# Ashish424/G.P.U-PathTracer

Hardware: AMD Instinct MI355X
Metric: Mrays/sec, cornell_dragon 1920x1080 (+ achieved GB/s against the memory roofline) (higher is better)
Workload: dtype f32; 1 GPU; cornell_dragon_800k (800032 tris) 1920x1080 depth 4 diff + reference 8-sphere room, 16 spp per step; kernel=auto, parallelism=1 GPU, closed_scene=True

## Files before the change

g.p.u-pathtracer_amd/__init__.py:

```python
from . import _abi
from ._abi import (Camera, Params, Sphere, Material, Counters, BuildParams, DenoiseParams, MAT_DIFF, MAT_METAL, MAT_SPEC, MAT_REFR,
                   FLAG_METAL_LITERAL_W, FLAG_WRITE_RGBA, FLAG_FACE_FORWARD, FLAG_COSINE_DIFF, FLAG_GLASS_FIX, FLAG_RUSSIAN_ROULETTE, FLAG_MISS_KEEPS_PATH, FLAG_RR_CPU_TRACER, FLAG_NEE, FLAGS_SMALLPT, FLAGS_CPU_TRACER, KERNEL_AUTO, KERNEL_MEGA_BVH2,
                   KERNEL_PERSISTENT, KERNEL_WAVEFRONT, OPT_KERNEL, OPT_COUNTERS, OPT_TIMING, OPT_BATCH, OPT_TOP_NODES, OPT_OCCUPANCY, OPT_LDS_STACK, OPT_WALK, OPT_LEAF_MAX, OPT_TRI_TEST, OPT_REFILL, OPT_VOTE_NODE, OPT_VOTE_REC, OPT_WAVE_BATCH, OPT_SPHERE_LDS, OPT_BUILD_ALGO, OPT_REBUILD, OPT_PRESPLIT, OPT_WAVE_BLOCKS, OPT_OVERLAP, OPT_OPTIMIZE, OPT_WAVE_SAMPLES,
                   OPT_FIRST_WALK, OPT_PACKET_STACK, OPT_FUSE_STAGES)
from .host import (Mesh, Bvh, write_image, save_checkpoint, load_checkpoint, frame_hash, reference_spheres, default_camera, default_params, scene_mesh)
from .tracer import PathTracer, PtError, DeviceBuffer, algorithmic_bytes, DENOISE_DEFAULTS

__all__ = [n for n in dir() if not n.startswith("_")]
```

g.p.u-pathtracer_amd/_abi.py:

```python
import ctypes as C
import os

_HERE = os.path.dirname(os.path.abspath(__file__))
PTMI_PATH = os.environ.get("PT_LIBPTMI") or os.path.join(_HERE, "csrc", "libptmi.so")
PTHOST_PATH = os.path.join(_HERE, "host", "libpthost.so")


class Camera(C.Structure):
    _fields_ = [("pos", C.c_float * 3), ("front", C.c_float * 3), ("right", C.c_float * 3),
                ("up", C.c_float * 3), ("dist", C.c_float), ("aspect", C.c_float),
                ("fov", C.c_float), ("_pad", C.c_float)]


class Sphere(C.Structure):
    _fields_ = [("pos_rad", C.c_float * 4), ("emi", C.c_float * 3), ("col", C.c_float * 3),
                ("mat", C.c_int32)]


class Material(C.Structure):
    _fields_ = [("col", C.c_float * 3), ("emi", C.c_float * 3), ("mat", C.c_int32), ("phong_expo", C.c_float)]


class DenoiseParams(C.Structure):
    _fields_ = [("width", C.c_int32), ("height", C.c_int32), ("iterations", C.c_int32),
# ... 22 lines not shown

class BuildParams(C.Structure):
    _fields_ = [("max_leaf_size", C.c_int32), ("min_leaf_size", C.c_int32), ("max_depth", C.c_int32),
                ("n_bins", C.c_int32), ("sah_node_cost", C.c_float), ("sah_tri_cost", C.c_float),
                ("split_alpha", C.c_float), ("n_spatial_bins", C.c_int32), ("optimize_passes", C.c_int32)]


class BvhStats(C.Structure):
    _fields_ = [("n_inner", C.c_uint64), ("n_leaves", C.c_uint64), ("n_tri_refs", C.c_uint64),
                ("max_depth", C.c_uint32), ("sah_cost", C.c_float), ("build_ms", C.c_double),
                ("opt_cost_before", C.c_float), ("opt_cost_after", C.c_float)]


MAT_DIFF, MAT_METAL, MAT_SPEC, MAT_REFR = 0, 1, 2, 3
FLAG_METAL_LITERAL_W = 1 << 0
FLAG_WRITE_RGBA = 1 << 1
FLAG_FACE_FORWARD, FLAG_COSINE_DIFF, FLAG_GLASS_FIX, FLAG_RUSSIAN_ROULETTE, FLAG_MISS_KEEPS_PATH = 1 << 2, 1 << 3, 1 << 4, 1 << 5, 1 << 6
FLAG_RR_CPU_TRACER = 1 << 7
FLAG_NEE = 1 << 8
FLAGS_SMALLPT = FLAG_FACE_FORWARD | FLAG_COSINE_DIFF | FLAG_RUSSIAN_ROULETTE | FLAG_MISS_KEEPS_PATH
FLAGS_CPU_TRACER = FLAG_FACE_FORWARD | FLAG_COSINE_DIFF | FLAG_RR_CPU_TRACER | FLAG_MISS_KEEPS_PATH
KERNEL_AUTO, KERNEL_MEGA_BVH2, KERNEL_PERSISTENT, KERNEL_WAVEFRONT = 0, 1, 3, 5
OPT_KERNEL, OPT_COUNTERS, OPT_TIMING, OPT_BATCH, OPT_TOP_NODES, OPT_OCCUPANCY, OPT_LDS_STACK, OPT_WALK, OPT_LEAF_MAX, OPT_TRI_TEST, OPT_REFILL, OPT_VOTE_NODE, OPT_VOTE_REC, OPT_WAVE_BATCH, OPT_SPHERE_LDS, OPT_BUILD_ALGO, OPT_REBUILD, OPT_PRESPLIT, OPT_WAVE_BLOCKS, OPT_OVERLAP, OPT_OPTIMIZE, OPT_WAVE_SAMPLES = 1, 2, 3, 4, 5, 6, 7, 8, 9, 10, 11, 12, 13, 14, 15, 16, 17, 18, 19, 21, 24, 25
OPT_FIRST_WALK, OPT_PACKET_STACK, OPT_FUSE_STAGES = 26, 27, 28

_vp, _sz, _i, _u32 = C.c_void_p, C.c_size_t, C.c_int, C.c_uint32
PTMI_SYMBOLS = [
    ("pt_abi_version", _i, []),
    ("pt_device_count", _i, []),
    ("pt_create", _i, [_i, C.POINTER(_vp)]),
    ("pt_destroy", _i, [_vp]),
    ("pt_last_error", C.c_char_p, [_vp]),
    ("pt_set_stream", _i, [_vp, _vp]),
    ("pt_set_option", _i, [_vp, _i, _i]),
    ("pt_sync", _i, [_vp]),
    ("pt_malloc", _i, [_vp, _sz, C.POINTER(_vp)]),
    ("pt_free", _i, [_vp, _vp]),
    ("pt_memset", _i, [_vp, _vp, _i, _sz]),
    ("pt_download", _i, [_vp, _vp, _vp, _sz]),
    ("pt_upload", _i, [_vp, _vp, _vp, _sz]),
    ("pt_upload_bvh", _i, [_vp, _vp, _sz, _vp, _sz, _vp, _sz]),
    ("pt_upload_spheres", _i, [_vp, C.POINTER(Sphere), _sz]),
    ("pt_render", _i, [_vp, _vp, _vp, C.POINTER(Camera), C.POINTER(Params), _u32]),
    ("pt_trace_rays", _i, [_vp, _vp, _sz, _i, _vp, _vp, _vp]),
    ("pt_render_aux", _i, [_vp, C.POINTER(Camera), C.POINTER(Params), _vp, _vp, _vp, _vp]),
    ("pt_denoise", _i, [_vp, C.POINTER(DenoiseParams), _vp, _vp, _vp, _vp, _vp, _vp]),
    ("pt_build_bvh", _i, [_vp, _vp, C.c_size_t, _vp, C.c_size_t]),
# ... 78 lines not shown
```

g.p.u-pathtracer_amd/csrc/pt_ctx.h:

```cpp
#pragma once
#include <hip/hip_runtime.h>

#include <algorithm>
#include <cstdint>
#include <string>
#include <vector>

#include "../../include/ptmi.h"
#include "pt_kernels.h"

#ifndef PT_FIRST_WALK_DEFAULT
#define PT_FIRST_WALK_DEFAULT 1
#endif

struct pt_ctx {
    int device = 0;
    hipStream_t own_stream = nullptr;
    hipStream_t stream = nullptr;
    std::string err;
    float4* d_nodes = nullptr;
    float4* d_tris = nullptr;
    pt_sphere_d* d_spheres = nullptr;
    int* d_tri_matid = nullptr;
    float4* d_mat_table = nullptr;
// ... 28 lines not shown
    int opt_presplit = 0;
    int opt_optimize = 0;
    double opt_cost[2] = {0.0, 0.0};
    int opt_rebuild = 0;
    int opt_build_algo = 1;
    int opt_sph_lds = 1;
    int opt_vote_node = 1, opt_vote_rec = 1;
    int opt_refill = 8;
    int opt_top = 64;
    int opt_occ = 6;
    int opt_lstk = 16;
    int opt_walk = 2;
    int opt_leaf_max = 2;
    int opt_tri_test = 0;
    bool records_woop = false;
    void* d_wave = nullptr;
    size_t wave_bytes = 0;
    int opt_wave_batch = 16;
    int opt_wave_samples = 16;
    int opt_wave_blocks = 8;
    int opt_first_walk = PT_FIRST_WALK_DEFAULT;
    int opt_packet_stack = PT_PACKET_STACK_MAX;
    int opt_fuse_stages = 1;
    struct AutoPick {
        static constexpr int TRIALS = 4, PENDING = 4, DECIDED = 5;
        uint64_t key = 0;
        int phase = 0;
        int choice = PT_KERNEL_PERSISTENT;
        hipEvent_t e[2 * TRIALS] = {nullptr, nullptr, nullptr, nullptr, nullptr, nullptr, nullptr, nullptr};
        float ms[2] = {0.f, 0.f};
        uint64_t used = 0;
    };
    static constexpr int N_PICKS = 8;
    AutoPick picks[N_PICKS];
    int pick_last = -1;
    uint64_t pick_tick = 0;
    uint64_t scene_gen = 0;
    uint64_t geom_gen = 0;
    hipEvent_t geom_ev = nullptr;
    struct Refit {
        uint64_t scene_gen = 0;
        const float4* items = nullptr;
        void* d_mem = nullptr;
        int4* bin_list = nullptr;
        int4* wide_list = nullptr;
        float* bin_box = nullptr;
// ... 94 lines not shown
```

g.p.u-pathtracer_amd/csrc/pt_k_wave.hip:

```cpp
#include "pt_ctx.h"

__device__ __forceinline__ int wf_block_rank(bool keep, int& total, int* s_cnt) {
    const unsigned long long m = __ballot(keep);
    const int w = threadIdx.x >> 6;
    const int in_wave = (int)__builtin_amdgcn_mbcnt_hi((uint32_t)(m >> 32), __builtin_amdgcn_mbcnt_lo((uint32_t)m, 0u));
    if ((threadIdx.x & 63) == 0) s_cnt[w] = __popcll(m);
    __syncthreads();
    int base = 0, tot = 0;
#pragma unroll
    for (int k = 0; k < PT_BLOCK / 64; k++) {
        const int c = s_cnt[k];
        if (k < w) base += c;
        tot += c;
    }
    total = tot;
    return base + in_wave;
}

__device__ __forceinline__ void wf_sphere_table() {
    if (threadIdx.x < 11 * PT_KSPHERES) {
        PT_KARGS(K);
        const float v = ((const __attribute__((address_space(4))) float*)&K.ksph[0])[threadIdx.x];
        ((float*)s_dyn)[threadIdx.x] = v;
        if (threadIdx.x % 11 < 4) ((float*)s_dyn)[88 + 4 * (threadIdx.x / 11) + threadIdx.x % 11] = v;
    }
    __syncthreads();
}

__global__ void __launch_bounds__(256) k_wf_prepare(const KParams P) {
    for (uint32_t i = threadIdx.x; i < P.spp; i += 256) P.wf.hashes[i] = pt_wang64(P.frame + i);
    for (uint32_t i = threadIdx.x; i < P.wf.queues_words; i += 256) P.wf.queues_all[i] = 0u;
}

__device__ __forceinline__ bool wf_slot_pixel(const KParams& P, uint32_t slot, uint32_t& s_idx, int& px, int& py) {
    if (slot >= P.wf.n_slots) return false;
    return pt_slot_pixel(P, slot, s_idx, px, py);
}

template <bool COUNT, int OCC, int LSTK, bool FIRST>
__global__ void __launch_bounds__(PT_BLOCK, OCC) k_wf_extend(const KParams P) {
    const int tid = threadIdx.x;
    const int lane = tid & 63;
    TravOverflow<LSTK> stk_ovf;
    TravStack<LSTK, PT_BLOCK> stk(__builtin_amdgcn_readfirstlane(tid & ~63), stk_ovf);
    const bool cull = P.cull != 0;
    const uint32_t n_regions = (uint32_t)P.wf.n_regions;
    const uint32_t shard_regions = (n_regions + PT_SHARDS - 1) / PT_SHARDS;
    const int batch = P.batch;

    uint32_t next = 0, end = 0;
    bool empty = false;
    int shard = (int)(blockIdx.x & (PT_SHARDS - 1));

    bool live = false;
    uint32_t idx = 0;
    v3 o = V3(0.f, 0.f, 0.f), d = V3(0.f, 0.f, 0.f);
    TravState ts;
    ts.idx = ts.idy = ts.idz = ts.oodx = ts.oody = ts.oodz = 0.f;
    ts.node = PT_SENTINEL; ts.leaf = 0; ts.sp = 0;
    ts.h.t = PT_F32_MAX; ts.h.tri = -1; ts.h.rec = 0;
    TravCount tc;
    tc.inner = tc.tris = tc.leaves = 0;
// ... 9 lines not shown
            uint32_t served = 0;
            for (int round = 0; round < 8 && served < (uint32_t)n_idle; round++) {
                if (next == end) {
                    bool got = false;
                    for (int tries = 0; tries < PT_SHARDS && !got; tries++) {
                        uint32_t k = 0;
                        if (lane == 0) k = atomicAdd(P.wf.queue + shard * PT_SHARD_STRIDE, 1u);
                        k = (uint32_t)__builtin_amdgcn_readfirstlane((int)k);
                        const uint32_t r = k * PT_SHARDS + (uint32_t)shard;
                        if (k < shard_regions && r < n_regions) {
                            next = r * PT_REGION;
                            if (FIRST) end = min(next + (uint32_t)PT_REGION, P.wf.n_slots);
                            else end = next + (uint32_t)__builtin_amdgcn_readfirstlane(P.wf.cnt_in[r]);
                            got = true;
                        } else {
                            shard = (shard + 1) & (PT_SHARDS - 1);
                        }
                    }
                    if (!got) { empty = true; break; }
                }
                const uint32_t take = min((uint32_t)n_idle - served, end - next);
                if (!live && rank >= served && rank < served + take) {
                    idx = next + (rank - served);
                    if (FIRST) {
                        uint32_t s_idx = 0;
                        int px = 0, py = 0;
                        if (wf_slot_pixel(P, idx, s_idx, px, py)) {
                            PathState ps;
                            path_begin_hashed(P, px, py, (uint64_t)((uint32_t)py * (uint32_t)P.W + (uint32_t)px), P.wf.hashes[s_idx], ps);
                            o = ps.o;
                            d = ps.d;
                            live = true;
                        }
                    } else {
                        const float4 a = pt_sld4(P.wf.ray0_in + idx), b = pt_sld4(P.wf.ray1_in + idx);
                        o = V3(a.x, a.y, a.z);
                        d = V3(a.w, b.x, b.y);
                        live = true;
                    }
                    if (live) trav_begin(ts, o, d, stk, P.sc.wide_root);
                }
                next += take;
                served += take;
            }
            if (COUNT && served) { it_begin++; act_begin += served; }
        }
        const unsigned long long busy = __ballot(live);
        if (!busy) {
            if (empty) break;
            continue;
        }
        const int n_dead = empty ? 64 - __popcll(busy) : 0;
        if (live) {
            const bool fin = trav_run_wide<COUNT, true, false, true>(ts, P.sc, o, d, cull, stk, tc, n_dead, batch);
            if (fin) {
                pt_sst2(P.wf.hit + idx, make_float2(ts.h.t, __int_as_float(ts.h.rec)));
                live = false;
                if (COUNT) n_rays++;
            }
        }
    }

    if (COUNT) {
        const uint32_t a = wave_sum_u32(n_rays), b = wave_sum_u32(tc.inner), c = wave_sum_u32(tc.tris), dd = wave_sum_u32(tc.leaves);
        const uint32_t w_it_node = wave_sum_u32(tc.it_node), w_act_node = wave_sum_u32(tc.act_node);
        const uint32_t w_it_rec = wave_sum_u32(tc.it_rec), w_act_rec = wave_sum_u32(tc.act_rec);
        const uint32_t w_ovf = wave_sum_u32(stk.n_ovf);
        if (lane == 0) {
            atomicAdd(&P.counters[0], (unsigned long long)a);
            atomicAdd(&P.counters[1], (unsigned long long)b);
            atomicAdd(&P.counters[2], (unsigned long long)c);
            atomicAdd(&P.counters[3], (unsigned long long)dd);
            atomicAdd(&P.counters[6], (unsigned long long)w_it_node);
            atomicAdd(&P.counters[7], (unsigned long long)w_act_node);
            atomicAdd(&P.counters[8], (unsigned long long)w_it_rec);
            atomicAdd(&P.counters[9], (unsigned long long)w_act_rec);
            atomicAdd(&P.counters[12], (unsigned long long)it_begin);
            atomicAdd(&P.counters[13], (unsigned long long)act_begin);
            atomicAdd(&P.counters[14], (unsigned long long)it_loop);
            atomicAdd(&P.counters[15], (unsigned long long)w_ovf);
        }
    }
}

template <bool COUNT>
__global__ void __launch_bounds__(PT_BLOCK, 8) k_wf_extend_packet(const KParams P) {
    const uint32_t n_groups = P.wf.n_slots / 64u;
    const uint32_t stride = gridDim.x * (uint32_t)(PT_BLOCK / 64);
    TravCount tc;
    tc.inner = tc.tris = tc.leaves = 0;
    tc.it_node = tc.act_node = tc.it_rec = tc.act_rec = 0;
    uint32_t n_rays = 0, n_walked = 0;
    for (uint32_t group = (uint32_t)__builtin_amdgcn_readfirstlane((int)(blockIdx.x * (PT_BLOCK / 64) + (threadIdx.x >> 6)));
         group < n_groups; group += stride) {
        const uint32_t slot = group * 64u + (threadIdx.x & 63u);
        uint32_t s_idx = 0;
        int px = 0, py = 0;
        v3 o = V3(0.f, 0.f, 0.f), d = V3(0.f, 0.f, 0.f);
        const bool in = wf_slot_pixel(P, slot, s_idx, px, py);
// ... 47 lines not shown
        return false;
    }
    v3 col;
    const bool done = LAST ? true : path_shade_hit(P, ps, h, sh, tri_n, col, 0, NEE ? req : nullptr);
    if (LAST) col = path_last_emission(P, ps, h, sh, 0);
    const v3 e = done ? col : ps.accu;
    if (FIRST) {
        pt_sst3(smp, V3(0.f + e.x, 0.f + e.y, 0.f + e.z));
    } else if (!(e.x == 0.f) || !(e.y == 0.f) || !(e.z == 0.f)) {
        smp[0] += e.x; smp[1] += e.y; smp[2] += e.z;
    }
    return !done;
}

template <int LP>
__device__ __forceinline__ void wf_fold_region(const KParams& P, uint32_t region) {
    if (threadIdx.x >= 64) return;
    uint32_t s_idx = 0;
    int px = 0, py = 0;
    const bool in = wf_slot_pixel(P, region * PT_REGION + (threadIdx.x / LP) * (4u * LP), s_idx, px, py);
    pt_fold_pixel_grouped<LP>(P, in, in ? (size_t)py * (size_t)P.W + (size_t)px : 0, (int)(threadIdx.x % LP));
}

template <bool COUNT, bool NEE, bool FIRST, bool LAST = false, int FOLD = 0>
__global__ void __launch_bounds__(PT_BLOCK) k_wf_shade(const KParams P) {
    __shared__ int s_cnt[PT_BLOCK / 64];
    __shared__ int s_cnt2[PT_BLOCK / 64];
    const uint32_t region = blockIdx.x;
    const int n_in = FIRST ? PT_REGION : P.wf.cnt_in[region];
    const bool last = LAST || P.wf.bounce + 1 >= P.depth;
    if (n_in == 0) {
        if (!last && threadIdx.x == 0) P.wf.cnt_out[region] = 0;
        if (NEE && threadIdx.x == 0) P.wf.s_cnt[region] = 0;
        if constexpr (FOLD > 0) wf_fold_region<FOLD>(P, region);
        return;
    }
    wf_sphere_table();
    const size_t i = (size_t)region * PT_REGION + threadIdx.x;
    bool have = (int)threadIdx.x < n_in;
    bool alive = false, tri_hit = false;
    PathState ps;
    NeeReq req;
    req.want = false;
    uint32_t pix = 0, s_idx = 0;
    int px = 0, py = 0;
    if (FIRST) have = wf_slot_pixel(P, (uint32_t)i, s_idx, px, py);
    if (have) {
// ... 11 lines not shown
                ps.nee_mask = (pix >> 24) | ((sn >> 31) << 8);
                pix &= 0xffffffu;
                sn &= 0x7fffffffu;
            }
            s_idx = sn >> 12;
            ps.mask = V3(pt_sld1(P.wf.mask_in + i), pt_sld1(P.wf.mask_in + (size_t)P.wf.cap + i), pt_sld1(P.wf.mask_in + 2 * (size_t)P.wf.cap + i));
            ps.accu = V3(0.f, 0.f, 0.f);
            ps.depth = P.wf.bounce;
            ps.rng = pt_rng_init(P.wf.hashes[s_idx], (uint64_t)pix);
            ps.rng.n = sn & 0xfffu;
        }
        const float2 hh = pt_sld2(P.wf.hit + i);
        Hit h;
        h.t = hh.x;
        h.rec = __float_as_int(hh.y);
        h.tri = -1;
        tri_hit = h.t < PT_F32_MAX;
        if (tri_hit) {
            h.tri = 0;
            if (P.tri_matid) h.tri = __float_as_int(P.sc.nodes[h.rec].w);
        }
        alive = wf_shade_segment<NEE, FIRST, LAST>(P, ps, h, tri_hit, pt_sample_ptr(P, s_idx, (size_t)pix), &req);
    }
    if (COUNT) {
        const uint32_t nh = wave_sum_u32(tri_hit ? 1u : 0u), np = wave_sum_u32(have && !alive ? 1u : 0u);
        if ((threadIdx.x & 63) == 0) {
            atomicAdd(&P.counters[4], (unsigned long long)nh);
            atomicAdd(&P.counters[5], (unsigned long long)np);
        }
    }
    if (NEE) {
        int n_sh;
        const int rs = wf_block_rank(req.want, n_sh, s_cnt2);
        if (req.want) {
            const size_t j = (size_t)region * PT_REGION + (size_t)rs;
            P.wf.s_ray0[j] = make_float4(req.o.x, req.o.y, req.o.z, req.d.x);
            P.wf.s_ray1[j] = make_float4(req.d.y, req.d.z, __uint_as_float(pix), __uint_as_float(s_idx));
            P.wf.s_con[j] = make_float4(req.contrib.x, req.contrib.y, req.contrib.z, req.t_max);
        }
        if (threadIdx.x == 0) P.wf.s_cnt[region] = n_sh;
    }
    if (last) {
        if constexpr (FOLD > 0) {
            __syncthreads();
            wf_fold_region<FOLD>(P, region);
        }
        return;
    }
    int total;
    const int r = PT_SURVIVOR_RANK(P, alive, ps, total, s_cnt);
    if (alive) {
        const size_t j = (size_t)region * PT_REGION + (size_t)r;
        pt_sst4(P.wf.ray0_out + j, make_float4(ps.o.x, ps.o.y, ps.o.z, ps.d.x));
        pt_sst4(P.wf.ray1_out + j, make_float4(ps.d.y, ps.d.z, __uint_as_float(NEE ? (pix | ((ps.nee_mask & 0xffu) << 24)) : pix),
                                              __uint_as_float((s_idx << 12) | ps.rng.n | (NEE ? (ps.nee_mask >> 8) << 31 : 0u))));
        pt_sst1(P.wf.mask_out + j, ps.mask.x);
        pt_sst1(P.wf.mask_out + (size_t)P.wf.cap + j, ps.mask.y);
        pt_sst1(P.wf.mask_out + 2 * (size_t)P.wf.cap + j, ps.mask.z);
    }
    if (threadIdx.x == 0) P.wf.cnt_out[region] = total;
}

__global__ void __launch_bounds__(PT_BLOCK, 8) k_wf_extend_packet_shade(const KParams P) {
    __shared__ int s_cnt[PT_BLOCK / 64];
    wf_sphere_table();
    const uint32_t region = blockIdx.x;
    const size_t i = (size_t)region * PT_REGION + threadIdx.x;
    uint32_t s_idx = 0;
    int px = 0, py = 0;
    const bool have = wf_slot_pixel(P, (uint32_t)i, s_idx, px, py);
    const uint32_t pix = (uint32_t)py * (uint32_t)P.W + (uint32_t)px;
    PathState ps;
    ps.o = ps.d = V3(0.f, 0.f, 0.f);
    if (have) path_begin_hashed(P, px, py, (uint64_t)pix, P.wf.hashes[s_idx], ps);
    TravCount tc;
    tc.inner = tc.tris = tc.leaves = 0;
    tc.it_node = tc.act_node = tc.it_rec = tc.act_rec = 0;
    Hit h = trav_packet_wide<false>(P.sc, ps.o, ps.d, P.cull != 0, have, tc);
    bool alive = false;
    if (have) {
        const bool tri_hit = h.t < PT_F32_MAX;
        if (tri_hit && !P.tri_matid) h.tri = 0;
        alive = wf_shade_segment<false, true, false>(P, ps, h, tri_hit, pt_sample_ptr(P, s_idx, (size_t)pix), nullptr);
    }
    if (P.wf.bounce + 1 >= P.depth) return;
    int total;
    const int r = PT_SURVIVOR_RANK(P, alive, ps, total, s_cnt);
    if (alive) {
        const size_t j = (size_t)region * PT_REGION + (size_t)r;
        pt_sst4(P.wf.ray0_out + j, make_float4(ps.o.x, ps.o.y, ps.o.z, ps.d.x));
        pt_sst4(P.wf.ray1_out + j, make_float4(ps.d.y, ps.d.z, __uint_as_float(pix), __uint_as_float((s_idx << 12) | ps.rng.n)));
        pt_sst1(P.wf.mask_out + j, ps.mask.x);
        pt_sst1(P.wf.mask_out + (size_t)P.wf.cap + j, ps.mask.y);
        pt_sst1(P.wf.mask_out + 2 * (size_t)P.wf.cap + j, ps.mask.z);
    }
    if (threadIdx.x == 0) P.wf.cnt_out[region] = total;
}

__global__ void __launch_bounds__(PT_BLOCK) k_wf_resolve(const KParams P) {
    const int n_in = P.wf.s_cnt[blockIdx.x];
    if ((int)threadIdx.x >= n_in) return;
    const size_t i = (size_t)blockIdx.x * PT_REGION + threadIdx.x;
    const float4 c = P.wf.s_con[i];
    const float2 hh = P.wf.s_hit[i];
    if (hh.x < c.w) return;
    const float4 b = P.wf.s_ray1[i];
    const uint32_t pix = __float_as_uint(b.z), s_idx = __float_as_uint(b.w);
    float* smp = pt_sample_ptr(P, s_idx, (size_t)pix);
    smp[0] += c.x; smp[1] += c.y; smp[2] += c.z;
}

namespace ptmi {

struct WaveLayout {
    size_t n_regions, cap, b_ray, b_mask, b_hit, b_cnt, b_hash, q_words, b_q, b_nee, need;
    bool nee;
};
// ... 71 lines not shown
        P.wf.s_con = (float4*)(base + 2 * b_ray);
        P.wf.s_hit = (float2*)(base + 3 * b_ray);
        P.wf.s_cnt = (int*)(base + 3 * b_ray + b_hit);
    }

    hipStream_t st = c->stream;
    P.sc.n_top = 0;
    P.sph_tab = 0;
    P.batch = c->opt_wave_batch;
    P.wf.hit = hit;
    P.wf.hashes = hashes;
    P.wf.queues_all = queues;
    P.wf.queues_words = (uint32_t)q_words;
    P.wf.cap = (uint32_t)cap;
    P.wf.n_regions = (int)n_regions;
    P.wf.n_slots = (uint32_t)((size_t)work_tiles * 64);
    P.wf.bounce = 0;
    hipLaunchKernelGGL(k_wf_prepare, dim3(1), dim3(256), 0, st, P);
    HIP_TRY(c, hipGetLastError());
    if (stage_mark(c, PT_STAGE_GENERATE) != PT_OK) return PT_ERR_DEVICE;

    const size_t lds_ext = (size_t)(L.lstk == 24 ? 24 : 16) * PT_BLOCK * 4;
    const size_t lds_shade = 15 * PT_KSPHERES * 4;
#define PT_EXT(COUNT, OCC, LSTK, FIRST)                                                                           \
        do {                                                                                                      \
            int per_cu = 0;                                                                                       \
            if (allow_lds(k_wf_extend<COUNT, OCC, LSTK, FIRST>, lds_ext) != hipSuccess) return hipErrorInvalidValue; \
            if (hipOccupancyMaxActiveBlocksPerMultiprocessor(&per_cu, k_wf_extend<COUNT, OCC, LSTK, FIRST>, PT_BLOCK, lds_ext) != hipSuccess || per_cu < 1) \
                per_cu = 1;                                                                                       \
            per_cu = std::min(per_cu, blocks_per_cu);                                                             \
            hipLaunchKernelGGL((k_wf_extend<COUNT, OCC, LSTK, FIRST>), dim3((unsigned)std::min<size_t>((size_t)per_cu * L.n_cu, (size_t)Q.wf.n_regions)), \
                               dim3(PT_BLOCK), lds_ext, s, Q);                                                    \
        } while (0)
    const bool packet = c->opt_first_walk == 1 && 3 * c->wide_depth + 2 <= (uint32_t)c->opt_packet_stack;
    auto launch_extend = [&](const KParams& Q, bool first, hipStream_t s, int blocks_per_cu) -> hipError_t {
        if (first && packet) {
#ifdef PT_PACKET_RESIDENT_GRID
            const size_t n_blk = std::min<size_t>((size_t)Q.wf.n_regions, (size_t)8 * L.n_cu);
#else
            const size_t n_blk = L.count ? std::min<size_t>((size_t)Q.wf.n_regions, (size_t)8 * L.n_cu) : (size_t)Q.wf.n_regions;
#endif
            if (L.count) hipLaunchKernelGGL(k_wf_extend_packet<true>, dim3((unsigned)n_blk), dim3(PT_BLOCK), 0, s, Q);
            else hipLaunchKernelGGL(k_wf_extend_packet<false>, dim3((unsigned)n_blk), dim3(PT_BLOCK), 0, s, Q);
        } else if (first) {
            if (L.count) { if (L.lstk == 24) PT_EXT(true, 6, 24, true); else PT_EXT(true, 8, 16, true); }
            else { if (L.lstk == 24) PT_EXT(false, 6, 24, true); else PT_EXT(false, 8, 16, true); }
        } else {
            if (L.count) { if (L.lstk == 24) PT_EXT(true, 6, 24, false); else PT_EXT(true, 8, 16, false); }
            else { if (L.lstk == 24) PT_EXT(false, 6, 24, false); else PT_EXT(false, 8, 16, false); }
        }
        return hipGetLastError();
    };
#undef PT_EXT
#define PT_SHADE(COUNT, NEE, FIRST) \
        hipLaunchKernelGGL((k_wf_shade<COUNT, NEE, FIRST>), dim3((unsigned)Q.wf.n_regions), dim3(PT_BLOCK), lds_shade, s, Q)
    const bool fuse = c->opt_fuse_stages != 0 && !nee && !L.count;
    const bool fuse_first = fuse && packet;
    const int fold_lp = fuse && P.depth >= 2 && P.sgroup_log2 >= 2 && P.sgroup_log2 <= 4 && P.spp == (1u << P.sgroup_log2) ? (int)P.spp / 4 : 0;
    folded = fold_lp != 0;
    auto launch_shade = [&](const KParams& Q, bool first, hipStream_t s) -> hipError_t {
        if (!first && !nee && !L.count && Q.wf.bounce + 1 >= Q.depth) {
            const dim3 grid((unsigned)Q.wf.n_regions);
            if (fold_lp == 4) hipLaunchKernelGGL((k_wf_shade<false, false, false, true, 4>), grid, dim3(PT_BLOCK), lds_shade, s, Q);
            else if (fold_lp == 2) hipLaunchKernelGGL((k_wf_shade<false, false, false, true, 2>), grid, dim3(PT_BLOCK), lds_shade, s, Q);
            else if (fold_lp == 1) hipLaunchKernelGGL((k_wf_shade<false, false, false, true, 1>), grid, dim3(PT_BLOCK), lds_shade, s, Q);
            else hipLaunchKernelGGL((k_wf_shade<false, false, false, true>), grid, dim3(PT_BLOCK), lds_shade, s, Q);
            return hipGetLastError();
        }
        if (first) {
            if (nee) { if (L.count) PT_SHADE(true, true, true); else PT_SHADE(false, true, true); }
            else { if (L.count) PT_SHADE(true, false, true); else PT_SHADE(false, false, true); }
        } else {
            if (nee) { if (L.count) PT_SHADE(true, true, false); else PT_SHADE(false, true, false); }
            else { if (L.count) PT_SHADE(true, false, false); else PT_SHADE(false, false, false); }
        }
        return hipGetLastError();
    };
#undef PT_SHADE
    auto set_bounce = [&](KParams& Q, uint32_t b) {
        const int g = (int)(b & 1u);
        Q.wf.bounce = b;
        Q.wf.ray0_in = ray0[g]; Q.wf.ray1_in = ray1[g]; Q.wf.mask_in = mask[g]; Q.wf.cnt_in = cnt[g];
        Q.wf.ray0_out = ray0[g ^ 1]; Q.wf.ray1_out = ray1[g ^ 1]; Q.wf.mask_out = mask[g ^ 1]; Q.wf.cnt_out = cnt[g ^ 1];
    };

    for (uint32_t b = 0; b < P.depth; b++) {
        set_bounce(P, b);
        P.wf.queue = queues + (size_t)b * PT_SHARDS * PT_SHARD_STRIDE;
        if (b == 0 && fuse_first) {
            hipLaunchKernelGGL(k_wf_extend_packet_shade, dim3((unsigned)n_regions), dim3(PT_BLOCK), lds_shade, st, P);
            HIP_TRY(c, hipGetLastError());
            if (stage_mark(c, PT_STAGE_EXTEND) != PT_OK) return PT_ERR_DEVICE;
            continue;
        }
        HIP_TRY(c, launch_extend(P, b == 0, st, c->opt_wave_blocks));
        if (stage_mark(c, PT_STAGE_EXTEND) != PT_OK) return PT_ERR_DEVICE;
        HIP_TRY(c, launch_shade(P, b == 0, st));
        if (stage_mark(c, PT_STAGE_SHADE) != PT_OK) return PT_ERR_DEVICE;
        if (nee) {
            KParams S = P;
            S.wf.ray0_in = P.wf.s_ray0; S.wf.ray1_in = P.wf.s_ray1; S.wf.cnt_in = P.wf.s_cnt; S.wf.hit = P.wf.s_hit;
            S.wf.queue = queues + ((size_t)P.depth + b) * PT_SHARDS * PT_SHARD_STRIDE;
            HIP_TRY(c, launch_extend(S, false, st, c->opt_wave_blocks));
            if (stage_mark(c, PT_STAGE_EXTEND) != PT_OK) return PT_ERR_DEVICE;
            hipLaunchKernelGGL(k_wf_resolve, dim3((unsigned)n_regions), dim3(PT_BLOCK), 0, st, P);
            HIP_TRY(c, hipGetLastError());
            if (stage_mark(c, PT_STAGE_SHADE) != PT_OK) return PT_ERR_DEVICE;
        }
    }
    return PT_OK;
}

}
```

g.p.u-pathtracer_amd/csrc/pt_walks.h:

```cpp
#pragma once

extern __shared__ float4 s_dyn[];

#ifndef PT_NODE_STEP_HOOK
#define PT_NODE_STEP_HOOK(sc, a, w)
#endif
#ifndef PT_WIDE_VOTE_NODE
#define PT_WIDE_VOTE_NODE 1
#define PT_WIDE_VOTE_REC 1
#endif
#ifndef PT_WALK_DECL_HOOK
#define PT_WALK_DECL_HOOK()
#define PT_NODE_END_HOOK(sc, cur)
#define PT_WALK_EXIT_HOOK()
#endif

struct TravState {
    float idx, idy, idz, oodx, oody, oodz;
    int node, leaf, sp;
    Hit h;
};

__device__ __forceinline__ int pt_lane_fresh() {
    int l;
// ... 252 lines not shown
    for (int k = 0; k < 4; k++) {
        const pt_f2 tx = pt_fma2(pt_mk2((float)((nx >> (8 * k)) & 0xffu), (float)((fx >> (8 * k)) & 0xffu)), pt_mk2(sx, sx), pt_mk2(bx, bx));
        const pt_f2 ty = pt_fma2(pt_mk2((float)((ny >> (8 * k)) & 0xffu), (float)((fy >> (8 * k)) & 0xffu)), pt_mk2(sy, sy), pt_mk2(by, by));
        const pt_f2 tz = pt_fma2(pt_mk2((float)((nz >> (8 * k)) & 0xffu), (float)((fz >> (8 * k)) & 0xffu)), pt_mk2(sz, sz), pt_mk2(bz, bz));
        const float tmin = fmaxf(fmaxf(fmaxf(tx.x, ty.x), tz.x), 0.0f);
        const float tmax = fminf(fminf(fminf(tx.y, ty.y), tz.y), t_max);
        const bool hit = tmin <= tmax;
        key[k] = hit ? ((__float_as_uint(tmin) & 0x7ffffffcu) | (uint32_t)k) : 0xffffffffu;
    }
}

__device__ __forceinline__ void wide_sort4(uint32_t key[4]) {
#define PT_CE(i, j) { const uint32_t lo_ = min(key[i], key[j]), hi_ = max(key[i], key[j]); key[i] = lo_; key[j] = hi_; }
    PT_CE(0, 1) PT_CE(2, 3) PT_CE(0, 2) PT_CE(1, 3) PT_CE(1, 2)
#undef PT_CE
}

__device__ __forceinline__ void wide_node_keys(const WideNode& w, float idx, float idy, float idz, float oodx, float oody, float oodz,
                                               float t_max, uint32_t key[4]) {
    wide_node_keys_raw(w, idx, idy, idz, oodx, oody, oodz, t_max, key);
    wide_sort4(key);
}

template <bool COUNT, bool DYN, bool WOOP, bool AHEAD = false, class STK>
__device__ __forceinline__ bool trav_run_wide(TravState& s, const KScene& sc, v3 o, v3 d, bool cull, STK& stk,
                                              TravCount& tc, int n_dead, int batch) {
    int cur = s.node, sp = s.sp;
    Hit h = s.h;
    const float idx = s.idx, idy = s.idy, idz = s.idz, oodx = s.oodx, oody = s.oody, oodz = s.oodz;
    PT_WALK_DECL_HOOK();
    for (;;) {
        const bool live = cur != PT_SENTINEL;
        const bool is_node = live && cur >= 0;
        const int n_live = __popcll(__ballot(live));
        if (n_live == 0) break;
        if (DYN && 64 - n_live - n_dead >= batch) break;
        const int n_node = __popcll(__ballot(is_node));
        const bool node_phase = PT_WIDE_VOTE_NODE * n_node >= PT_WIDE_VOTE_REC * (n_live - n_node);
        if (COUNT && pt_first_active_lane()) {
            if (node_phase) { tc.it_node++; tc.act_node += n_node; }
            else { tc.it_rec++; tc.act_rec += n_live - n_node; }
        }
        if (!live || is_node != node_phase) continue;
        const int a = cur >= 0 ? cur : (~cur & ~3);
        if (cur >= 0) {
            const WideNode w = wide_node_load(sc, a);
            if (COUNT) tc.inner++;
// ... 23 lines not shown
                q0 = p_[0]; q1 = p_[1]; q2 = p_[2];
                x0 = x1 = x2 = make_float4(0.f, 0.f, 0.f, 0.f);
                if ((~cur & 3) != 0) { x0 = p_[4]; x1 = p_[5]; x2 = p_[6]; }
                asm volatile("" : "+v"(q0.x), "+v"(q0.y), "+v"(q0.z), "+v"(q0.w), "+v"(q1.x), "+v"(q1.y), "+v"(q1.z), "+v"(q1.w),
                                  "+v"(q2.x), "+v"(q2.y), "+v"(q2.z), "+v"(q2.w), "+v"(x0.x), "+v"(x0.y), "+v"(x0.z), "+v"(x0.w),
                                  "+v"(x1.x), "+v"(x1.y), "+v"(x1.z), "+v"(x1.w), "+v"(x2.x), "+v"(x2.y), "+v"(x2.z), "+v"(x2.w));
            } else
            pt_ld4x3(sc.nodes + a, q0, q1, q2);
            if (COUNT) tc.tris++;
            float t;
            int id;
            bool last;
            if (WOOP) {
                const float4 qw = sc.nodes[a + 3];
                t = pt_woop_intersect(q0, q1, q2, V3(qw.x, qw.y, qw.z), o, d, cull);
                id = __float_as_int(qw.w) >> 1;
                last = (__float_as_int(qw.w) & 1) != 0;
            } else {
                const v3 v0 = V3(q0.x, q0.y, q0.z), e1 = V3(q1.x, q1.y, q1.z), e2 = V3(q2.x, q2.y, q2.z);
                t = pt_mt_intersect(v0, e1, e2, o, d, cull);
                id = __float_as_int(q0.w);
                last = __float_as_int(q1.w) != 0;
            }
            if (t > 0.0f && (t < h.t || (t == h.t && h.tri != -1 && id < h.tri))) {
                h.t = t;
                h.tri = id;
                h.rec = a;
            }
            if (!WOOP) {
                int aa = a;
                if (AHEAD && !last) {
                    aa += 4;
                    if (COUNT) tc.tris++;
                    const float t2 = pt_mt_intersect(V3(x0.x, x0.y, x0.z), V3(x1.x, x1.y, x1.z), V3(x2.x, x2.y, x2.z), o, d, cull);
                    const int id2 = __float_as_int(x0.w);
                    last = __float_as_int(x1.w) != 0;
                    if (t2 > 0.0f && (t2 < h.t || (t2 == h.t && h.tri != -1 && id2 < h.tri))) {
                        h.t = t2;
                        h.tri = id2;
                        h.rec = aa;
                    }
                }
                while (!last) {
                    aa += 4;
                    float4 r0, r1, r2;
                    pt_ld4x3(sc.nodes + aa, r0, r1, r2);
// ... 225 lines not shown
```

g.p.u-pathtracer_amd/csrc/ptmi.hip:

```cpp
#include <hip/hip_runtime.h>

#include <algorithm>
#include <cmath>
#include <cstdio>
#include <cstring>
#include <string>
#include <vector>

#include "pt_ctx.h"
#include "pt_scene_build.h"

static_assert(sizeof(pt_sphere) == 44, "pt_sphere must match the reference Sphere (44 B)");
static_assert(sizeof(pt_sphere_d) == sizeof(pt_sphere), "device sphere mirror");
static_assert(sizeof(pt_params) == 104 && sizeof(pt_camera) == 64 && sizeof(pt_counters) == 48, "ABI struct sizes (tests/test_host_and_abi.py)");

namespace ptmi {
thread_local std::string g_err;
}
using namespace ptmi;

namespace ptmi {
static int tree_cost_impl(pt_ctx* c, double* node_visits, double* tri_tests);

struct TreeState {
// ... 266 lines not shown
        case PT_OPT_LDS_STACK:
            if (value != 0 && value != 16 && value != 24) return fail(c, PT_ERR_INVALID, "pt_set_option: LDS stack must be 0 (all 72 entries in LDS), 16 or 24 entries");
            c->opt_lstk = value;
            return PT_OK;
        case PT_OPT_REFILL:
            if (value < 1 || value > 64) return fail(c, PT_ERR_INVALID, "pt_set_option: refill must be 1..64");
            c->opt_refill = value;
            return PT_OK;
        case PT_OPT_BATCH:
            if (value < 1 || value > 64) return fail(c, PT_ERR_INVALID, "pt_set_option: batch must be 1..64");
            c->opt_batch = value;
            return PT_OK;
        case PT_OPT_FIRST_WALK:
            if (value != 0 && value != 1) return fail(c, PT_ERR_INVALID, "pt_set_option: first walk must be 0 (per lane) or 1 (wave-wide packets)");
            c->opt_first_walk = value;
            return PT_OK;
        case PT_OPT_PACKET_STACK:
            if (value < 2 || value > PT_PACKET_STACK_MAX) return fail(c, PT_ERR_INVALID, "pt_set_option: packet stack must be 2..72 entries");
            c->opt_packet_stack = value;
            return PT_OK;
        case PT_OPT_FUSE_STAGES:
            if (value != 0 && value != 1) return fail(c, PT_ERR_INVALID, "pt_set_option: fuse stages must be 0 (separate launches) or 1");
            c->opt_fuse_stages = value;
            return PT_OK;
        default: return fail(c, PT_ERR_INVALID, "pt_set_option: unknown option");
    }
}

int pt_sync(pt_ctx* c) {
    if (!c) return fail(nullptr, PT_ERR_INVALID, "null ctx");
    HIP_TRY(c, hipSetDevice(c->device));
    HIP_TRY(c, hipStreamSynchronize(c->stream));
    return PT_OK;
}

int pt_malloc(pt_ctx* c, size_t bytes, void** out) {
    if (!c || !out || bytes == 0) return fail(c, PT_ERR_INVALID, "pt_malloc: bad argument");
    HIP_TRY(c, hipSetDevice(c->device));
    HIP_TRY(c, hipMalloc(out, bytes));
    return PT_OK;
}
int pt_free(pt_ctx* c, void* p) {
    if (!c) return fail(nullptr, PT_ERR_INVALID, "null ctx");
    HIP_TRY(c, hipSetDevice(c->device));
    HIP_TRY(c, hipStreamSynchronize(c->stream));
    HIP_TRY(c, hipFree(p));
// ... 650 lines not shown
```

include/ptmi.h:

```cpp
#ifndef PTMI_H
#define PTMI_H

#include <stddef.h>
#include <stdint.h>

#ifdef __cplusplus
extern "C" {
#endif

#define PTMI_ABI_VERSION 3

typedef struct pt_ctx pt_ctx;

typedef enum pt_status {
    PT_OK = 0,
    PT_ERR_INVALID = -1,
    PT_ERR_DEVICE = -2,
    PT_ERR_NO_SCENE = -3,
    PT_ERR_NOMEM = -4,
    PT_ERR_UNSUPPORTED = -5
} pt_status;

enum { PT_MAT_DIFF = 0, PT_MAT_METAL = 1, PT_MAT_SPEC = 2, PT_MAT_REFR = 3 };

// ... 23 lines not shown
    PT_OPT_COUNTERS = 2,
    PT_OPT_TIMING = 3,
    PT_OPT_BATCH = 4,
    PT_OPT_TOP_NODES = 5,
    PT_OPT_OCCUPANCY = 6,
    PT_OPT_LDS_STACK = 7,
    PT_OPT_WALK = 8,
    PT_OPT_REFILL = 11,
    PT_OPT_VOTE_NODE = 12,
    PT_OPT_VOTE_REC = 13,
    PT_OPT_WAVE_BATCH = 14,
    PT_OPT_SPHERE_LDS = 15,
    PT_OPT_WAVE_BLOCKS = 19,
    PT_OPT_WAVE_SAMPLES = 25,
    PT_OPT_FIRST_WALK = 26,
    PT_OPT_PACKET_STACK = 27,
    PT_OPT_OVERLAP = 21,
    PT_OPT_BUILD_ALGO = 16,
    PT_OPT_REBUILD = 17,
    PT_OPT_OPTIMIZE = 24,
    PT_OPT_PRESPLIT = 18,
    PT_OPT_TRI_TEST = 10,
    PT_OPT_LEAF_MAX = 9,
    PT_OPT_FUSE_STAGES = 28
};

typedef struct pt_camera {
    float pos[3];
    float front[3];
    float right[3];
    float up[3];
    float dist;
    float aspect;
    float fov;
    float _pad;
} pt_camera;

typedef struct pt_sphere {
    float pos_rad[4];
    float emi[3];
    float col[3];
    int32_t mat;
} pt_sphere;

typedef struct pt_params {
    int32_t width, height;
    uint32_t depth;
// ... 101 lines not shown
```

Baseline: 16350 Mrays/s.

## Use any-hit occlusion traversal for the last bounce when triangles are non-emissive

```diff
diff --git a/g.p.u-pathtracer_amd/__init__.py b/g.p.u-pathtracer_amd/__init__.py
--- a/g.p.u-pathtracer_amd/__init__.py
+++ b/g.p.u-pathtracer_amd/__init__.py
@@ -2,7 +2,7 @@
 from ._abi import (Camera, Params, Sphere, Material, Counters, BuildParams, DenoiseParams, MAT_DIFF, MAT_METAL, MAT_SPEC, MAT_REFR,
                    FLAG_METAL_LITERAL_W, FLAG_WRITE_RGBA, FLAG_FACE_FORWARD, FLAG_COSINE_DIFF, FLAG_GLASS_FIX, FLAG_RUSSIAN_ROULETTE, FLAG_MISS_KEEPS_PATH, FLAG_RR_CPU_TRACER, FLAG_NEE, FLAGS_SMALLPT, FLAGS_CPU_TRACER, KERNEL_AUTO, KERNEL_MEGA_BVH2,
                    KERNEL_PERSISTENT, KERNEL_WAVEFRONT, OPT_KERNEL, OPT_COUNTERS, OPT_TIMING, OPT_BATCH, OPT_TOP_NODES, OPT_OCCUPANCY, OPT_LDS_STACK, OPT_WALK, OPT_LEAF_MAX, OPT_TRI_TEST, OPT_REFILL, OPT_VOTE_NODE, OPT_VOTE_REC, OPT_WAVE_BATCH, OPT_SPHERE_LDS, OPT_BUILD_ALGO, OPT_REBUILD, OPT_PRESPLIT, OPT_WAVE_BLOCKS, OPT_OVERLAP, OPT_OPTIMIZE, OPT_WAVE_SAMPLES,
-                   OPT_FIRST_WALK, OPT_PACKET_STACK, OPT_FUSE_STAGES)
+                   OPT_FIRST_WALK, OPT_PACKET_STACK, OPT_FUSE_STAGES, OPT_LAST_ANYHIT)
 from .host import (Mesh, Bvh, write_image, save_checkpoint, load_checkpoint, frame_hash, reference_spheres, default_camera, default_params, scene_mesh)
 from .tracer import PathTracer, PtError, DeviceBuffer, algorithmic_bytes, DENOISE_DEFAULTS
 
diff --git a/g.p.u-pathtracer_amd/_abi.py b/g.p.u-pathtracer_amd/_abi.py
--- a/g.p.u-pathtracer_amd/_abi.py
+++ b/g.p.u-pathtracer_amd/_abi.py
@@ -68,7 +68,7 @@
 FLAGS_CPU_TRACER = FLAG_FACE_FORWARD | FLAG_COSINE_DIFF | FLAG_RR_CPU_TRACER | FLAG_MISS_KEEPS_PATH
 KERNEL_AUTO, KERNEL_MEGA_BVH2, KERNEL_PERSISTENT, KERNEL_WAVEFRONT = 0, 1, 3, 5
 OPT_KERNEL, OPT_COUNTERS, OPT_TIMING, OPT_BATCH, OPT_TOP_NODES, OPT_OCCUPANCY, OPT_LDS_STACK, OPT_WALK, OPT_LEAF_MAX, OPT_TRI_TEST, OPT_REFILL, OPT_VOTE_NODE, OPT_VOTE_REC, OPT_WAVE_BATCH, OPT_SPHERE_LDS, OPT_BUILD_ALGO, OPT_REBUILD, OPT_PRESPLIT, OPT_WAVE_BLOCKS, OPT_OVERLAP, OPT_OPTIMIZE, OPT_WAVE_SAMPLES = 1, 2, 3, 4, 5, 6, 7, 8, 9, 10, 11, 12, 13, 14, 15, 16, 17, 18, 19, 21, 24, 25
-OPT_FIRST_WALK, OPT_PACKET_STACK, OPT_FUSE_STAGES = 26, 27, 28
+OPT_FIRST_WALK, OPT_PACKET_STACK, OPT_FUSE_STAGES, OPT_LAST_ANYHIT = 26, 27, 28, 29
 
 _vp, _sz, _i, _u32 = C.c_void_p, C.c_size_t, C.c_int, C.c_uint32
 PTMI_SYMBOLS = [
diff --git a/g.p.u-pathtracer_amd/csrc/pt_ctx.h b/g.p.u-pathtracer_amd/csrc/pt_ctx.h
--- a/g.p.u-pathtracer_amd/csrc/pt_ctx.h
+++ b/g.p.u-pathtracer_amd/csrc/pt_ctx.h
@@ -74,6 +74,7 @@
     int opt_first_walk = PT_FIRST_WALK_DEFAULT;
     int opt_packet_stack = PT_PACKET_STACK_MAX;
     int opt_fuse_stages = 1;
+    int opt_last_anyhit = 1;
     struct AutoPick {
         static constexpr int TRIALS = 4, PENDING = 4, DECIDED = 5;
         uint64_t key = 0;
diff --git a/g.p.u-pathtracer_amd/csrc/pt_k_wave.hip b/g.p.u-pathtracer_amd/csrc/pt_k_wave.hip
--- a/g.p.u-pathtracer_amd/csrc/pt_k_wave.hip
+++ b/g.p.u-pathtracer_amd/csrc/pt_k_wave.hip
@@ -37,7 +37,7 @@
     return pt_slot_pixel(P, slot, s_idx, px, py);
 }
 
-template <bool COUNT, int OCC, int LSTK, bool FIRST>
+template <bool COUNT, int OCC, int LSTK, bool FIRST, bool ANY = false>
 __global__ void __launch_bounds__(PT_BLOCK, OCC) k_wf_extend(const KParams P) {
     const int tid = threadIdx.x;
     const int lane = tid & 63;
@@ -93,6 +93,7 @@
                 const uint32_t take = min((uint32_t)n_idle - served, end - next);
                 if (!live && rank >= served && rank < served + take) {
                     idx = next + (rank - served);
+                    float bound = PT_F32_MAX;
                     if (FIRST) {
                         uint32_t s_idx = 0;
                         int px = 0, py = 0;
@@ -105,11 +106,13 @@
                         }
                     } else {
                         const float4 a = pt_sld4(P.wf.ray0_in + idx), b = pt_sld4(P.wf.ray1_in + idx);
+                        if (ANY) bound = pt_sld1((const float*)(P.wf.hit + idx));
                         o = V3(a.x, a.y, a.z);
                         d = V3(a.w, b.x, b.y);
                         live = true;
                     }
                     if (live) trav_begin(ts, o, d, stk, P.sc.wide_root);
+                    if (ANY) ts.h.t = bound < PT_F32_MAX ? __uint_as_float(__float_as_uint(bound) + 1u) : bound;
                 }
                 next += take;
                 served += take;
@@ -123,9 +126,10 @@
         }
         const int n_dead = empty ? 64 - __popcll(busy) : 0;
         if (live) {
-            const bool fin = trav_run_wide<COUNT, true, false, true>(ts, P.sc, o, d, cull, stk, tc, n_dead, batch);
+            const bool fin = trav_run_wide<COUNT, true, false, true, ANY>(ts, P.sc, o, d, cull, stk, tc, n_dead, batch);
             if (fin) {
-                pt_sst2(P.wf.hit + idx, make_float2(ts.h.t, __int_as_float(ts.h.rec)));
+                if (ANY) { if (ts.h.t == 0.0f) pt_sst1((float*)(P.wf.hit + idx), 0.0f); }
+                else pt_sst2(P.wf.hit + idx, make_float2(ts.h.t, __int_as_float(ts.h.rec)));
                 live = false;
                 if (COUNT) n_rays++;
             }
@@ -146,6 +150,7 @@
             atomicAdd(&P.counters[7], (unsigned long long)w_act_node);
             atomicAdd(&P.counters[8], (unsigned long long)w_it_rec);
             atomicAdd(&P.counters[9], (unsigned long long)w_act_rec);
+            if (ANY) atomicAdd(&P.counters[11], (unsigned long long)a);
             atomicAdd(&P.counters[12], (unsigned long long)it_begin);
             atomicAdd(&P.counters[13], (unsigned long long)act_begin);
             atomicAdd(&P.counters[14], (unsigned long long)it_loop);
@@ -239,7 +244,14 @@
     pt_fold_pixel_grouped<LP>(P, in, in ? (size_t)py * (size_t)P.W + (size_t)px : 0, (int)(threadIdx.x % LP));
 }
 
-template <bool COUNT, bool NEE, bool FIRST, bool LAST = false, int FOLD = 0>
+__device__ __forceinline__ float2 wf_sphere_bound(const KParams& P, const PathState& ps) {
+    Hit none;
+    none.t = PT_F32_MAX; none.tri = -1; none.rec = 0;
+    const SceneHit sh = pt_closest_sphere(P, ps.o, ps.d, none, 0);
+    return make_float2(sh.t, __int_as_float(sh.sph_id));
+}
+
+template <bool COUNT, bool NEE, bool FIRST, bool LAST = false, int FOLD = 0, bool BOUND = false>
 __global__ void __launch_bounds__(PT_BLOCK) k_wf_shade(const KParams P) {
     __shared__ int s_cnt[PT_BLOCK / 64];
     __shared__ int s_cnt2[PT_BLOCK / 64];
@@ -297,6 +309,8 @@
         }
         alive = wf_shade_segment<NEE, FIRST, LAST>(P, ps, h, tri_hit, pt_sample_ptr(P, s_idx, (size_t)pix), &req);
     }
+    float2 bound = make_float2(PT_F32_MAX, __int_as_float(-1));
+    if (BOUND && alive) bound = wf_sphere_bound(P, ps);
     if (COUNT) {
         const uint32_t nh = wave_sum_u32(tri_hit ? 1u : 0u), np = wave_sum_u32(have && !alive ? 1u : 0u);
         if ((threadIdx.x & 63) == 0) {
@@ -332,10 +346,58 @@
         pt_sst1(P.wf.mask_out + j, ps.mask.x);
         pt_sst1(P.wf.mask_out + (size_t)P.wf.cap + j, ps.mask.y);
         pt_sst1(P.wf.mask_out + 2 * (size_t)P.wf.cap + j, ps.mask.z);
+        if (BOUND) pt_sst2(P.wf.hit + j, bound);
     }
     if (threadIdx.x == 0) P.wf.cnt_out[region] = total;
 }
 
+template <bool COUNT, int FOLD>
+__global__ void __launch_bounds__(PT_BLOCK) k_wf_shade_last_any(const KParams P) {
+    const uint32_t region = blockIdx.x;
+    const int n_in = P.wf.cnt_in[region];
+    if (n_in == 0) {
+        if constexpr (FOLD > 0) wf_fold_region<FOLD>(P, region);
+        return;
+    }
+    wf_sphere_table();
+    const size_t i = (size_t)region * PT_REGION + threadIdx.x;
+    const bool have = (int)threadIdx.x < n_in;
+    bool tri_hit = false;
+    if (have) {
+        const float4 b = pt_sld4(P.wf.ray1_in + i);
+        const float2 hh = pt_sld2(P.wf.hit + i);
+        const v3 mask = V3(pt_sld1(P.wf.mask_in + i), pt_sld1(P.wf.mask_in + (size_t)P.wf.cap + i), pt_sld1(P.wf.mask_in + 2 * (size_t)P.wf.cap + i));
+        const uint32_t pix = __float_as_uint(b.z), s_idx = __float_as_uint(b.w) >> 12;
+        float* smp = pt_sample_ptr(P, s_idx, (size_t)pix);
+        const int sph = __float_as_int(hh.y);
+        tri_hit = hh.x == 0.0f;
+        if (!tri_hit && sph >= 0) {
+            const float* t = (const float*)s_dyn + 11 * sph;
+            const v3 e = vadd(V3(0.f, 0.f, 0.f), vmul(mask, V3(t[4], t[5], t[6])));
+            if (!(e.x == 0.f) || !(e.y == 0.f) || !(e.z == 0.f)) { smp[0] += e.x; smp[1] += e.y; smp[2] += e.z; }
+        } else if (!tri_hit) {
+            PT_KARGS(K);
+            if (K.flags & PT_FLAG_MISS_KEEPS_PATH) {
+                smp[0] += mask.x * K.bk[0]; smp[1] += mask.y * K.bk[1]; smp[2] += mask.z * K.bk[2];
+            } else {
+                smp[0] = K.bk[0]; smp[1] = K.bk[1]; smp[2] = K.bk[2];
+            }
+        }
+    }
+    if (COUNT) {
+        const uint32_t nh = wave_sum_u32(tri_hit ? 1u : 0u), np = wave_sum_u32(have ? 1u : 0u);
+        if ((threadIdx.x & 63) == 0) {
+            atomicAdd(&P.counters[4], (unsigned long long)nh);
+            atomicAdd(&P.counters[5], (unsigned long long)np);
+        }
+    }
+    if constexpr (FOLD > 0) {
+        __syncthreads();
+        wf_fold_region<FOLD>(P, region);
+    }
+}
+
+template <bool BOUND>
 __global__ void __launch_bounds__(PT_BLOCK, 8) k_wf_extend_packet_shade(const KParams P) {
     __shared__ int s_cnt[PT_BLOCK / 64];
     wf_sphere_table();
@@ -359,6 +421,8 @@
         alive = wf_shade_segment<false, true, false>(P, ps, h, tri_hit, pt_sample_ptr(P, s_idx, (size_t)pix), nullptr);
     }
     if (P.wf.bounce + 1 >= P.depth) return;
+    float2 bound = make_float2(PT_F32_MAX, __int_as_float(-1));
+    if (BOUND && alive) bound = wf_sphere_bound(P, ps);
     int total;
     const int r = PT_SURVIVOR_RANK(P, alive, ps, total, s_cnt);
     if (alive) {
@@ -368,6 +432,7 @@
         pt_sst1(P.wf.mask_out + j, ps.mask.x);
         pt_sst1(P.wf.mask_out + (size_t)P.wf.cap + j, ps.mask.y);
         pt_sst1(P.wf.mask_out + 2 * (size_t)P.wf.cap + j, ps.mask.z);
+        if (BOUND) pt_sst2(P.wf.hit + j, bound);
     }
     if (threadIdx.x == 0) P.wf.cnt_out[region] = total;
 }
@@ -485,18 +550,18 @@
 
     const size_t lds_ext = (size_t)(L.lstk == 24 ? 24 : 16) * PT_BLOCK * 4;
     const size_t lds_shade = 15 * PT_KSPHERES * 4;
-#define PT_EXT(COUNT, OCC, LSTK, FIRST)                                                                           \
+#define PT_EXT(COUNT, OCC, LSTK, FIRST, ANY)                                                                         \
         do {                                                                                                      \
             int per_cu = 0;                                                                                       \
-            if (allow_lds(k_wf_extend<COUNT, OCC, LSTK, FIRST>, lds_ext) != hipSuccess) return hipErrorInvalidValue; \
-            if (hipOccupancyMaxActiveBlocksPerMultiprocessor(&per_cu, k_wf_extend<COUNT, OCC, LSTK, FIRST>, PT_BLOCK, lds_ext) != hipSuccess || per_cu < 1) \
+            if (allow_lds(k_wf_extend<COUNT, OCC, LSTK, FIRST, ANY>, lds_ext) != hipSuccess) return hipErrorInvalidValue; \
+            if (hipOccupancyMaxActiveBlocksPerMultiprocessor(&per_cu, k_wf_extend<COUNT, OCC, LSTK, FIRST, ANY>, PT_BLOCK, lds_ext) != hipSuccess || per_cu < 1) \
                 per_cu = 1;                                                                                       \
             per_cu = std::min(per_cu, blocks_per_cu);                                                             \
-            hipLaunchKernelGGL((k_wf_extend<COUNT, OCC, LSTK, FIRST>), dim3((unsigned)std::min<size_t>((size_t)per_cu * L.n_cu, (size_t)Q.wf.n_regions)), \
+            hipLaunchKernelGGL((k_wf_extend<COUNT, OCC, LSTK, FIRST, ANY>), dim3((unsigned)std::min<size_t>((size_t)per_cu * L.n_cu, (size_t)Q.wf.n_regions)), \
                                dim3(PT_BLOCK), lds_ext, s, Q);                                                    \
         } while (0)
     const bool packet = c->opt_first_walk == 1 && 3 * c->wide_depth + 2 <= (uint32_t)c->opt_packet_stack;
-    auto launch_extend = [&](const KParams& Q, bool first, hipStream_t s, int blocks_per_cu) -> hipError_t {
+    auto launch_extend = [&](const KParams& Q, bool first, hipStream_t s, int blocks_per_cu, bool any = false) -> hipError_t {
         if (first && packet) {
 #ifdef PT_PACKET_RESIDENT_GRID
             const size_t n_blk = std::min<size_t>((size_t)Q.wf.n_regions, (size_t)8 * L.n_cu);
@@ -506,22 +571,45 @@
             if (L.count) hipLaunchKernelGGL(k_wf_extend_packet<true>, dim3((unsigned)n_blk), dim3(PT_BLOCK), 0, s, Q);
             else hipLaunchKernelGGL(k_wf_extend_packet<false>, dim3((unsigned)n_blk), dim3(PT_BLOCK), 0, s, Q);
         } else if (first) {
-            if (L.count) { if (L.lstk == 24) PT_EXT(true, 6, 24, true); else PT_EXT(true, 8, 16, true); }
-            else { if (L.lstk == 24) PT_EXT(false, 6, 24, true); else PT_EXT(false, 8, 16, true); }
+            if (L.count) { if (L.lstk == 24) PT_EXT(true, 6, 24, true, false); else PT_EXT(true, 8, 16, true, false); }
+            else { if (L.lstk == 24) PT_EXT(false, 6, 24, true, false); else PT_EXT(false, 8, 16, true, false); }
+        } else if (any) {
+            if (L.count) { if (L.lstk == 24) PT_EXT(true, 6, 24, false, true); else PT_EXT(true, 8, 16, false, true); }
+            else { if (L.lstk == 24) PT_EXT(false, 6, 24, false, true); else PT_EXT(false, 8, 16, false, true); }
         } else {
-            if (L.count) { if (L.lstk == 24) PT_EXT(true, 6, 24, false); else PT_EXT(true, 8, 16, false); }
-            else { if (L.lstk == 24) PT_EXT(false, 6, 24, false); else PT_EXT(false, 8, 16, false); }
+            if (L.count) { if (L.lstk == 24) PT_EXT(true, 6, 24, false, false); else PT_EXT(true, 8, 16, false, false); }
+            else { if (L.lstk == 24) PT_EXT(false, 6, 24, false, false); else PT_EXT(false, 8, 16, false, false); }
         }
         return hipGetLastError();
     };
 #undef PT_EXT
 #define PT_SHADE(COUNT, NEE, FIRST) \
         hipLaunchKernelGGL((k_wf_shade<COUNT, NEE, FIRST>), dim3((unsigned)Q.wf.n_regions), dim3(PT_BLOCK), lds_shade, s, Q)
+#define PT_SHADE_BOUND(COUNT, FIRST) \
+        hipLaunchKernelGGL((k_wf_shade<COUNT, false, FIRST, false, 0, true>), dim3((unsigned)Q.wf.n_regions), dim3(PT_BLOCK), lds_shade, s, Q)
+#define PT_SHADE_ANY(COUNT, FOLD) \
+        hipLaunchKernelGGL((k_wf_shade_last_any<COUNT, FOLD>), dim3((unsigned)Q.wf.n_regions), dim3(PT_BLOCK), lds_shade, s, Q)
     const bool fuse = c->opt_fuse_stages != 0 && !nee && !L.count;
     const bool fuse_first = fuse && packet;
     const int fold_lp = fuse && P.depth >= 2 && P.sgroup_log2 >= 2 && P.sgroup_log2 <= 4 && P.spp == (1u << P.sgroup_log2) ? (int)P.spp / 4 : 0;
     folded = fold_lp != 0;
+    const bool tri_dark = P.tri_emi[0] == 0.f && P.tri_emi[1] == 0.f && P.tri_emi[2] == 0.f;
+    const bool anyhit = (L.count ? c->opt_last_anyhit == 2 : c->opt_last_anyhit >= 1) && P.depth >= 2 && !nee && !P.tri_matid && tri_dark &&
+                        P.sc.n_spheres <= PT_KSPHERES && !c->records_woop;
     auto launch_shade = [&](const KParams& Q, bool first, hipStream_t s) -> hipError_t {
+        if (anyhit && Q.wf.bounce + 1 >= Q.depth) {
+            if (L.count) PT_SHADE_ANY(true, 0);
+            else if (fold_lp == 4) PT_SHADE_ANY(false, 4);
+            else if (fold_lp == 2) PT_SHADE_ANY(false, 2);
+            else if (fold_lp == 1) PT_SHADE_ANY(false, 1);
+            else PT_SHADE_ANY(false, 0);
+            return hipGetLastError();
+        }
+        if (anyhit && Q.wf.bounce + 2 == Q.depth) {
+            if (first) { if (L.count) PT_SHADE_BOUND(true, true); else PT_SHADE_BOUND(false, true); }
+            else { if (L.count) PT_SHADE_BOUND(true, false); else PT_SHADE_BOUND(false, false); }
+            return hipGetLastError();
+        }
         if (!first && !nee && !L.count && Q.wf.bounce + 1 >= Q.depth) {
             const dim3 grid((unsigned)Q.wf.n_regions);
             if (fold_lp == 4) hipLaunchKernelGGL((k_wf_shade<false, false, false, true, 4>), grid, dim3(PT_BLOCK), lds_shade, s, Q);
@@ -540,6 +628,8 @@
         return hipGetLastError();
     };
 #undef PT_SHADE
+#undef PT_SHADE_BOUND
+#undef PT_SHADE_ANY
     auto set_bounce = [&](KParams& Q, uint32_t b) {
         const int g = (int)(b & 1u);
         Q.wf.bounce = b;
@@ -551,12 +641,13 @@
         set_bounce(P, b);
         P.wf.queue = queues + (size_t)b * PT_SHARDS * PT_SHARD_STRIDE;
         if (b == 0 && fuse_first) {
-            hipLaunchKernelGGL(k_wf_extend_packet_shade, dim3((unsigned)n_regions), dim3(PT_BLOCK), lds_shade, st, P);
+            if (anyhit && P.depth == 2) hipLaunchKernelGGL(k_wf_extend_packet_shade<true>, dim3((unsigned)n_regions), dim3(PT_BLOCK), lds_shade, st, P);
+            else hipLaunchKernelGGL(k_wf_extend_packet_shade<false>, dim3((unsigned)n_regions), dim3(PT_BLOCK), lds_shade, st, P);
             HIP_TRY(c, hipGetLastError());
             if (stage_mark(c, PT_STAGE_EXTEND) != PT_OK) return PT_ERR_DEVICE;
             continue;
         }
-        HIP_TRY(c, launch_extend(P, b == 0, st, c->opt_wave_blocks));
+        HIP_TRY(c, launch_extend(P, b == 0, st, c->opt_wave_blocks, anyhit && b + 1 == P.depth));
         if (stage_mark(c, PT_STAGE_EXTEND) != PT_OK) return PT_ERR_DEVICE;
         HIP_TRY(c, launch_shade(P, b == 0, st));
         if (stage_mark(c, PT_STAGE_SHADE) != PT_OK) return PT_ERR_DEVICE;
diff --git a/g.p.u-pathtracer_amd/csrc/pt_walks.h b/g.p.u-pathtracer_amd/csrc/pt_walks.h
--- a/g.p.u-pathtracer_amd/csrc/pt_walks.h
+++ b/g.p.u-pathtracer_amd/csrc/pt_walks.h
@@ -298,7 +298,7 @@
     wide_sort4(key);
 }
 
-template <bool COUNT, bool DYN, bool WOOP, bool AHEAD = false, class STK>
+template <bool COUNT, bool DYN, bool WOOP, bool AHEAD = false, bool ANY = false, class STK>
 __device__ __forceinline__ bool trav_run_wide(TravState& s, const KScene& sc, v3 o, v3 d, bool cull, STK& stk,
                                               TravCount& tc, int n_dead, int batch) {
     int cur = s.node, sp = s.sp;
@@ -368,6 +368,35 @@
                 id = __float_as_int(q0.w);
                 last = __float_as_int(q1.w) != 0;
             }
+            if constexpr (ANY) {
+                bool occ = t > 0.0f && t < h.t;
+                int aa = a;
+                if (AHEAD && !last && !occ) {
+                    aa += 4;
+                    if (COUNT) tc.tris++;
+                    const float t2 = pt_mt_intersect(V3(x0.x, x0.y, x0.z), V3(x1.x, x1.y, x1.z), V3(x2.x, x2.y, x2.z), o, d, cull);
+                    last = __float_as_int(x1.w) != 0;
+                    occ = t2 > 0.0f && t2 < h.t;
+                }
+                while (!last && !occ) {
+                    aa += 4;
+                    float4 r0, r1, r2;
+                    pt_ld4x3(sc.nodes + aa, r0, r1, r2);
+                    if (COUNT) tc.tris++;
+                    const float t2 = pt_mt_intersect(V3(r0.x, r0.y, r0.z), V3(r1.x, r1.y, r1.z), V3(r2.x, r2.y, r2.z), o, d, cull);
+                    last = __float_as_int(r1.w) != 0;
+                    occ = t2 > 0.0f && t2 < h.t;
+                }
+                if (occ) {
+                    h.t = 0.0f;
+                    cur = PT_SENTINEL;
+                } else {
+                    cur = stk.get(sp);
+                    sp--;
+                    if (COUNT && cur < 0 && cur != PT_SENTINEL) tc.leaves++;
+                }
+                continue;
+            }
             if (t > 0.0f && (t < h.t || (t == h.t && h.tri != -1 && id < h.tri))) {
                 h.t = t;
                 h.tri = id;
diff --git a/g.p.u-pathtracer_amd/csrc/ptmi.hip b/g.p.u-pathtracer_amd/csrc/ptmi.hip
--- a/g.p.u-pathtracer_amd/csrc/ptmi.hip
+++ b/g.p.u-pathtracer_amd/csrc/ptmi.hip
@@ -312,6 +312,10 @@
         case PT_OPT_FUSE_STAGES:
             if (value != 0 && value != 1) return fail(c, PT_ERR_INVALID, "pt_set_option: fuse stages must be 0 (separate launches) or 1");
             c->opt_fuse_stages = value;
+            return PT_OK;
+        case PT_OPT_LAST_ANYHIT:
+            if (value < 0 || value > 2) return fail(c, PT_ERR_INVALID, "pt_set_option: last any-hit must be 0 (off), 1 (product launches) or 2 (instrumented launches too)");
+            c->opt_last_anyhit = value;
             return PT_OK;
         default: return fail(c, PT_ERR_INVALID, "pt_set_option: unknown option");
     }
diff --git a/include/ptmi.h b/include/ptmi.h
--- a/include/ptmi.h
+++ b/include/ptmi.h
@@ -69,7 +69,8 @@
     PT_OPT_PRESPLIT = 18,
     PT_OPT_TRI_TEST = 10,
     PT_OPT_LEAF_MAX = 9,
-    PT_OPT_FUSE_STAGES = 28
+    PT_OPT_FUSE_STAGES = 28,
+    PT_OPT_LAST_ANYHIT = 29
 };
 
 typedef struct pt_camera {
```

Measured after the change: 16590 Mrays/s, median of 6. 1.5% higher.
